# ronnymilleo/amcpy

Hardware: AMD Instinct MI355X
Metric: IQ frames/sec (18 features, 2048-sample complex64) (higher is better)
Workload: dtype f32; 1 GPU; 6 mods x 26 SNR x 4096 frames x 2048 samples complex64 per GPU (BASELINE configs[1]), resident in HBM; one launch per step; frame_size=2048, kernel=amcx_features18_wave_kernel<2048>

## Files before the change

amcpy_amd/_lib.py:

```python
from __future__ import annotations

import ctypes as C
import os
from pathlib import Path

_HERE = Path(__file__).resolve().parent
LIB_PATH = Path(os.environ.get("AMCX_LIB", _HERE / "lib" / "libamcx.so"))

ABI_VERSION = 6
NUM_FEATURES = 18
VARIANT_AUTO, VARIANT_BLOCK, VARIANT_WAVE = 0, 1, 2
VARIANTS = {"auto": VARIANT_AUTO, "block": VARIANT_BLOCK, "wave": VARIANT_WAVE}
OK, EINVAL, ENOTSUP, EHIP, ENODEV, ENOMEM, EIO = 0, -1, -2, -3, -4, -5, -6
SRC_C64, SRC_C128, SRC_F32_SPLIT, SRC_F64_SPLIT = 0, 1, 2, 3


class UploadStats(C.Structure):
    _fields_ = [("frames", C.c_int64), ("source_bytes", C.c_int64), ("pcie_bytes", C.c_int64),
                ("chunks", C.c_int32), ("threads", C.c_int32), ("plane_major", C.c_int32), ("from_file", C.c_int32),
                ("seconds", C.c_double), ("seconds_staging", C.c_double), ("seconds_waiting", C.c_double),
                ("seconds_prepare", C.c_double), ("seconds_tail", C.c_double)]


class Placement(C.Structure):
    _fields_ = [("device", C.c_int32), ("numa_node", C.c_int32), ("n_cpus", C.c_int32), ("n_cpus_allowed", C.c_int32),
                ("first_cpu", C.c_int32), ("last_cpu", C.c_int32), ("pci_bus_id", C.c_char * 32)]


_i64, _i32, _vp, _fp = C.c_int64, C.c_int32, C.c_void_p, C.POINTER(C.c_float)
SIGNATURES = {
    "amcx_abi_version": (C.c_int, []),
    "amcx_strerror": (C.c_char_p, [C.c_int]),
    "amcx_last_hip_error": (C.c_char_p, []),
    "amcx_device_count": (C.c_int, []),
    "amcx_features18_c64": (C.c_int, [_vp, _i64, _i32, _i64, _vp, _i64, _vp]),
    "amcx_features18_c64_ex": (C.c_int, [_vp, _i64, _i32, _i64, _vp, _i64, _vp, _i32]),
    "amcx_features18_workspace_bytes": (_i64, [_i32, _i64, _i32]),
    "amcx_features18_c64_ws": (C.c_int, [_vp, _i64, _i32, _i64, _vp, _i64, _vp, _i32, _vp, _i64]),
    "amcx_features18_c64_host": (C.c_int, [_vp, _i64, _i32, _i64, _vp, _i64, _i32, _i32]),
    "amcx_features18_c128_host": (C.c_int, [_vp, _i64, _i32, _i64, _vp, _i64, _i32, _i32]),
    "amcx_ctx_create": (C.c_int, [_i32, C.POINTER(_vp)]),
    "amcx_ctx_destroy": (C.c_int, [_vp]),
    "amcx_ctx_features18_c64_host": (C.c_int, [_vp, _vp, _i64, _i32, _i64, _vp, _i64, _i32]),
    "amcx_ctx_features18_c128_host": (C.c_int, [_vp, _vp, _i64, _i32, _i64, _vp, _i64, _i32]),
    "amcx_ctx_features18_strided_host": (C.c_int, [_vp, _vp, _vp, _i32, _i64, _i64, _i32, _i64, _i64, _i64,
                                                   _vp, _i64, _i32]),
    "amcx_stage_host": (C.c_int, [_vp, _vp, _i32, _i64, _i64, _i32, _i64, _i64, _i64, _i64, _i64, _vp, _i64, _i32,
                                  C.POINTER(_i32), C.POINTER(_i32)]),
    "amcx_ctx_features18_strided_file": (C.c_int, [_vp, _i32, _i64, _i64, _i32, _i64, _i64, _i32, _i64, _i64, _i64,
                                                   _vp, _i64, _i32]),
    "amcx_stage_file": (C.c_int, [_i32, _i64, _i64, _i32, _i64, _i64, _i32, _i64, _i64, _i64, _i64, _i64, _vp, _i64, _i32,
                                  C.POINTER(_i32), C.POINTER(_i32)]),
    "amcx_ctx_configure": (C.c_int, [_vp, _i32, _i64, _i32]),
    "amcx_ctx_upload_stats": (C.c_int, [_vp, C.POINTER(UploadStats)]),
    "amcx_pack_planes_c64": (C.c_int, [_vp, _i32, _i32, _i64, _i64, _i64, _i32, _vp, _i64, _i32, _vp]),
    "amcx_kernel_name": (C.c_int, [_i32, _i32, C.c_char_p, _i32]),
    "amcx_probe_read_bw": (C.c_int, [_vp, _i64, _vp, _vp]),
    "amcx_probe_fma_rate": (C.c_int, [C.c_double, _vp, C.POINTER(C.c_double), C.POINTER(C.c_double)]),
    "amcx_device_pci_bus_id": (C.c_int, [_i32, C.c_char_p, _i32]),
    "amcx_numa_place": (C.c_int, [C.c_char_p, C.c_char_p, C.POINTER(_i32), C.POINTER(_i32), _i32, C.POINTER(_i32)]),
    "amcx_ctx_bind_cpus": (C.c_int, [_vp, C.POINTER(_i32), _i32]),
    "amcx_ctx_placement": (C.c_int, [_vp, C.POINTER(Placement)]),
    "amcx_group_stats_f32": (C.c_int, [_vp, _i64, _i64, _i64, _i32, _vp, _vp, _vp]),
    "amcx_select_scale_f32": (C.c_int, [_vp, _i64, _i64, _vp, _i32, _vp, _vp, _vp, _i64, _vp]),
    "amcx_group_stats_workspace_bytes": (_i64, [_i64, _i64, _i32]),
    "amcx_group_stats_ws_f32": (C.c_int, [_vp, _i64, _i64, _i64, _i32, _vp, _vp, _vp, _i64, _vp]),
    "amcx_standardize_workspace_bytes": (_i64, [_i64, _i32]),
    "amcx_standardize_fit_transform_f32": (C.c_int, [_vp, _i64, _i64, _i32, C.POINTER(_i32), _i32, _vp, _i64,
                                                     _vp, _vp, _vp, _i64, _vp]),
}

# ... 149 lines not shown
```

amcpy_amd/csrc/amcx.hip:

```cpp
#include "../../include/amcx.h"

#include <hip/hip_runtime.h>
#include <stdio.h>
#include <stdlib.h>
#include <string.h>
#include <chrono>
#include <new>

#include "amcx_block_kernel.h"
#include "amcx_stream_kernel.h"
#include "amcx_wave_kernel.h"
#include "amcx_quad_kernel.h"
#include "amcx_group_kernel.h"
#include "amcx_short_kernel.h"
#include "amcx_post_kernels.h"
#include "amcx_pack_kernel.h"
#include "amcx_upload.h"

namespace {

thread_local char g_hip_err[256] = "";

int hip_fail(hipError_t e, const char* what) {
  snprintf(g_hip_err, sizeof g_hip_err, "%s: %s", what, hipGetErrorString(e));
// ... 213 lines not shown
    case AMCX_OK: return "ok";
    case AMCX_EINVAL: return "invalid argument (null pointer, negative count, stride or frame_size out of range)";
    case AMCX_ENOTSUP: return "kernel variant does not support this frame_size";
    case AMCX_EHIP: return "HIP runtime error (see amcx_last_hip_error)";
    case AMCX_ENODEV: return "no usable gfx950 device";
    case AMCX_ENOMEM: return "device memory allocation failed";
    case AMCX_EIO: return "reading the container's file failed (see amcx_last_hip_error for the errno text)";
    default: return "unknown amcx error code";
  }
}

const char* amcx_last_hip_error(void) { return g_hip_err; }

int amcx_device_count(void) {
  int n = 0;
  hipError_t e = hipGetDeviceCount(&n);
  if (e == hipErrorNoDevice) return 0;
  if (e != hipSuccess) return hip_fail(e, "hipGetDeviceCount");
  int ok = 0;
  for (int d = 0; d < n; ++d) {
    hipDeviceProp_t p;
    if (hipGetDeviceProperties(&p, d) == hipSuccess && strncmp(p.gcnArchName, "gfx950", 6) == 0) ++ok;
  }
  return ok;
}

int64_t amcx_features18_workspace_bytes(int32_t frame_size, int64_t n_frames, int32_t variant) {
  if (n_frames < 0) return -1;
  const int v = resolve_variant(frame_size, variant);
  if (v < 0) return -1;
  if (v != AMCX_VARIANT_BLOCK || frame_size <= amcx::kBlockMaxN || n_frames == 0) return 0;
  const StreamPlan p = stream_plan(frame_size, n_frames);
  return (p.grid + (p.chirped ? 1 : 0)) * (int64_t)p.M * (int64_t)sizeof(float2);
}

int amcx_features18_c64_ws(const void* iq_dev, int64_t n_frames, int32_t frame_size,
                           int64_t row_stride_elems, float* out_dev, int64_t out_row_stride,
                           void* hip_stream, int32_t variant, void* workspace_dev, int64_t workspace_bytes) {
  if (n_frames < 0 || row_stride_elems < frame_size || out_row_stride < AMCX_NUM_FEATURES)
    return AMCX_EINVAL;
  const int v = resolve_variant(frame_size, variant);
  if (v < 0) return v;
  if (n_frames == 0) return AMCX_OK;
  if (iq_dev == nullptr || out_dev == nullptr) return AMCX_EINVAL;
  if ((reinterpret_cast<uintptr_t>(iq_dev) & 7u) || (reinterpret_cast<uintptr_t>(out_dev) & 3u))
    return AMCX_EINVAL;
  if (on_another_device(iq_dev) || on_another_device(out_dev)) return AMCX_EINVAL;
  hipStream_t stream = static_cast<hipStream_t>(hip_stream);
  const float2* iq = static_cast<const float2*>(iq_dev);
  if (v == AMCX_VARIANT_WAVE) {
    hipError_t e;
    if (frame_size == amcx::quad::kN)
      e = amcx::quad::launch_quad(iq, n_frames, row_stride_elems, out_dev, out_row_stride, stream, cu_count());
    else if (frame_size == amcx::group::G<8>::kN)
      e = amcx::group::launch_group<8>(iq, n_frames, row_stride_elems, out_dev, out_row_stride, stream, cu_count());
    else if (frame_size == amcx::group::G<16>::kN)
      e = amcx::group::launch_group<16>(iq, n_frames, row_stride_elems, out_dev, out_row_stride, stream, cu_count());
    else if (amcx::shortk::short_supports(frame_size))
      e = amcx::shortk::launch_short(iq, n_frames, frame_size, row_stride_elems, out_dev, out_row_stride, stream, cu_count());
    else
      e = amcx::launch_wave(iq, n_frames, frame_size, row_stride_elems, out_dev, out_row_stride, stream, cu_count());
    if (e != hipSuccess) return hip_fail(e, "wave kernel launch");
    return AMCX_OK;
  }
  if (workspace_dev != nullptr && on_another_device(workspace_dev)) return AMCX_EINVAL;
  return launch_block(iq, n_frames, frame_size, row_stride_elems, out_dev, out_row_stride, stream, workspace_dev,
                      workspace_bytes < 0 ? 0 : workspace_bytes);
}

int amcx_features18_c64_ex(const void* iq_dev, int64_t n_frames, int32_t frame_size,
                           int64_t row_stride_elems, float* out_dev, int64_t out_row_stride,
                           void* hip_stream, int32_t variant) {
  const int64_t want = n_frames > 0 && iq_dev != nullptr && out_dev != nullptr && row_stride_elems >= frame_size &&
                               out_row_stride >= AMCX_NUM_FEATURES
                           ? amcx_features18_workspace_bytes(frame_size, n_frames, variant) : 0;
  if (want <= 0)
    return amcx_features18_c64_ws(iq_dev, n_frames, frame_size, row_stride_elems, out_dev, out_row_stride, hip_stream,
                                  variant, nullptr, 0);
  hipStream_t st = static_cast<hipStream_t>(hip_stream);
  hipStreamCaptureStatus cap = hipStreamCaptureStatusNone;
  if (hipStreamIsCapturing(st, &cap) != hipSuccess) { (void)hipGetLastError(); cap = hipStreamCaptureStatusNone; }
  void* ws = nullptr;
  if (cap == hipStreamCaptureStatusNone && hipMallocAsync(&ws, (size_t)want, st) != hipSuccess) {
    (void)hipGetLastError();
    ws = nullptr;
  }
  if (ws == nullptr) {
    static const bool verbose = [] { const char* t = getenv("AMCX_VERBOSE"); return t != nullptr && t[0] != '\0' && t[0] != '0'; }();
    static std::atomic<bool> said{false};
    if (verbose && !said.exchange(true))
      fprintf(stderr, "amcx: frame_size %d runs the DFT by its definition (O(N^2)): %s; amcx_features18_c64_ws with %lld "
                      "bytes of workspace selects the FFT form\n", (int)frame_size,
              cap != hipStreamCaptureStatusNone ? "the stream is being captured" : "hipMallocAsync had no workspace", (long long)want);
  }
// ... 882 lines not shown
```

amcpy_amd/csrc/amcx_wave_kernel.h:

```cpp
#pragma once

#include <type_traits>
#include <utility>

#include "amcx_math.h"

#ifndef AMCX_PRIO_MASK
#define AMCX_PRIO_MASK 7
#endif
#define AMCX_PRIO_OF(b) ((AMCX_PRIO_MASK >> (b)) & 1)

namespace amcx {
namespace wave {

constexpr int kNumSums = 27;
constexpr int kStashStride = 33;

constexpr int kEx1StrideKK = 136, kEx1StrideB = 68;
constexpr int kEx2StrideK2 = 65;
constexpr int kExchangeBytes = (7 * kEx1StrideKK + kEx1StrideB + 64) * 8;
constexpr int kTw2Stride = 15 * 8;
constexpr int kTw3Row = 64 * 8;

template <int N>
struct Cfg {
  static_assert(N == 1024 || N == 2048 || N == 4096, "one wave per frame (128 ... 512: amcx_short_kernel.h; 8192 up: quad / group)");
  static constexpr bool kSplit = N == 4096;
  static constexpr int kFramesPerWave = N == 2048 ? 4 : 8;
  static constexpr int kFlushes = N == 4096 ? 2 : 1;
  static constexpr int kStashBytes = kFramesPerWave * kFlushes * kStashStride * 4;
  static constexpr int kTailChunk = 2;
  static constexpr int kRunFrames = kFramesPerWave;
  static constexpr int kWavesPerWG = kSplit ? 8 : 16;
  static constexpr int kThreads = 64 * kWavesPerWG;
  static constexpr int kTailFrames = kWavesPerWG * kFramesPerWave;
  static constexpr int kRows = N / 128;
  static constexpr int kHeldRows = kRows;
  static constexpr int kFftRows = kSplit ? 16 : kRows;
  static constexpr int kFftN = 128 * kFftRows;
  static constexpr int kPhases = kFftRows >= 8 ? kFftRows / 8 : 1;
  static constexpr int kT2Bytes = 8 * kPhases * kTw2Stride;
  static constexpr int kT3Bytes = kPhases * 2 * 7 * kTw3Row;
  static constexpr int kT4Bytes = kSplit ? 64 * 16 : 0;
  static constexpr int kTableBytes = kT2Bytes + kT3Bytes + kT4Bytes;
  static constexpr int kCounterOffset = kTableBytes + kWavesPerWG * (kExchangeBytes + kStashBytes);
  static constexpr int kLdsBytes = kCounterOffset + 16;
  static_assert(kLdsBytes <= 163840, "one workgroup per CU must fit in 160 KiB of LDS");
  static_assert(kFramesPerWave <= 64, "one frame per lane in the finaliser");
  static_assert(kSplit || 2 * kRows * 64 * 4 <= kExchangeBytes, "|x| parking must fit the exchange buffer");
// ... 483 lines not shown
      a[5] = __builtin_fma(A, Bh, a[5]);
      a[6] += AP;
      a[7] = __builtin_fma(Bh, P, a[7]);
      a[8] = __builtin_fma(AA, A, a[8]);
      a[9] = __builtin_fma(A, BB, a[9]);
      a[10] = __builtin_fma(AA, Bh, a[10]);
      a[11] = __builtin_fma(BB, Bh, a[11]);
      a[12] = __builtin_fma(AA, P, a[12]);
      a[13] = __builtin_fma(X4, P, a[13]);
      a[14] = __builtin_fma(AP, Bh, a[14]);
      if (u & 1) __builtin_amdgcn_sched_barrier(0);
    }
  }
#pragma unroll 1
  for (int off = 32; off >= 1; off >>= 1) {
#pragma unroll
    for (int k = 0; k < 15; ++k) a[k] += __shfl_xor(a[k], off, 64);
  }
#pragma unroll
  for (int k = 0; k < 15; ++k) t[k] = a[k];
}

template <int N>
__device__ __forceinline__ void wave_exact_cumulants(const float2* __restrict__ src, float sc, int h, int lane, bool mine,
                                                     float* __restrict__ dst_row) {
  double t[15];
  wave_exact_moments<N>(src, sc, lane, t);
  if (mine) {
    moment_features(t[0], t[1], t[2], t[3], t[4], t[5], t[6], t[7], t[8], t[9], t[10], t[11], t[12], t[13], t[14], (double)N,
                    [&](int j, int twice_order, double v) { dst_row[j] = (float)__builtin_ldexp(v, h * twice_order); });
  }
}

template <int N>
__device__ __forceinline__ void wave_body(
    const float2* __restrict__ iq, long long n_frames, long long row_stride,
    float* __restrict__ out, long long out_stride AMCX_STAMP_ARG) {
  using C = Cfg<N>;
  constexpr int R = C::kFftRows, ROWS = C::kHeldRows;
  constexpr int kWavesPerWG = C::kWavesPerWG, kThreads = C::kThreads, kTailFrames = C::kTailFrames;
  constexpr int kFramesPerWave = C::kFramesPerWave, kTailChunk = C::kTailChunk;
  extern __shared__ float4 amcx_wave_smem[];
  char* smem = reinterpret_cast<char*>(amcx_wave_smem);
  const int tid = threadIdx.x;
  const int lane = tid & 63;
  const int wave = __builtin_amdgcn_readfirstlane(tid >> 6);
  char* t2 = smem;
  char* t3 = smem + C::kT2Bytes;
  char* t4 = smem + C::kTableBytes - C::kT4Bytes;
  char* ex = smem + C::kTableBytes + wave * kExchangeBytes;
  float* stash = reinterpret_cast<float*>(smem + C::kTableBytes + kWavesPerWG * kExchangeBytes) +
                 wave * (kFramesPerWave * C::kFlushes * kStashStride);

  unsigned* const counters = reinterpret_cast<unsigned*>(smem + C::kCounterOffset);
  if (tid == 0) { counters[0] = 0; counters[1] = 0; }
  constexpr int kQ = C::kRunFrames;
  static_assert(kQ % kFramesPerWave == 0 && kFramesPerWave % kTailChunk == 0, "grabs stay inside a run");
  const long long n_wg = gridDim.x, wg = blockIdx.x;
  const long long full_runs = n_frames / kQ;
  const int rem_frames = (int)(n_frames - full_runs * kQ);
  const long long my_full = full_runs > wg ? (full_runs - wg - 1) / n_wg + 1 : 0;
  const long long slice_len = my_full * kQ + (rem_frames > 0 && full_runs % n_wg == wg ? rem_frames : 0);
  const long long body_len = slice_len > kTailFrames ? (slice_len - kTailFrames) / kFramesPerWave * kFramesPerWave : 0;
  const long long tail_len = slice_len - body_len;
  auto frame_of = [&](long long v) -> long long {
    const long long k = v / kQ;
    return (k * n_wg + wg) * kQ + (v - k * kQ);
  };

  build_fft_tables<C::kFftN>(t2, t3, tid, kThreads);
  if constexpr (C::kSplit) {
    for (int e = tid; e < 128; e += kThreads) {
      float sn, cs;
      sincospif((float)e * (1.0f / 2048.0f), &sn, &cs);
      reinterpret_cast<float2*>(t4)[e] = make_float2(cs, -sn);
    }
  }
  __syncthreads();

  const int kkL = lane >> 3, n3L = lane & 7;
  LaneAddr la;
  la.tw2 = t2 + kkL * kTw2Stride;
  la.tw3 = t3 + lane * 8;
  la.ex1_w = ex + lane * 8;
  la.ex1_r = ex + (kkL * kEx1StrideKK + (n3L & 1) * kEx1StrideB + (n3L >> 1)) * 8;
  la.ex2_w = ex + lane * 8;
  la.ex2_r = ex + (n3L * kEx2StrideK2 + kkL * 8) * 8;
  float* const a_lds = reinterpret_cast<float*>(ex) + lane;

#ifdef AMCX_WAVE_STAMPS
  unsigned long long stamp_acc[kStampSections] = {0, 0, 0, 0, 0, 0, 0, 0};
  unsigned long long stamp_last = __builtin_amdgcn_s_memtime();
  const unsigned long long real0 = __builtin_amdgcn_s_memrealtime();
#endif
  for (;;) {
    long long f0;
    int n_here;
    {
      unsigned got = 0;
      if (lane == 0) got = __hip_atomic_fetch_add(&counters[0], (unsigned)kFramesPerWave, __ATOMIC_RELAXED,
                                                  __HIP_MEMORY_SCOPE_WORKGROUP);
      got = __builtin_amdgcn_readfirstlane(got);
      if ((long long)got < body_len) {
        f0 = frame_of(got);
        const long long left = body_len - got;
        n_here = left < kFramesPerWave ? (int)left : kFramesPerWave;
      } else {
        unsigned t = 0;
        if (lane == 0) t = __hip_atomic_fetch_add(&counters[1], (unsigned)kTailChunk, __ATOMIC_RELAXED,
                                                  __HIP_MEMORY_SCOPE_WORKGROUP);
        t = __builtin_amdgcn_readfirstlane(t);
        if ((long long)t >= tail_len) break;
        f0 = frame_of(body_len + t);
        const long long left = tail_len - t;
        n_here = left < kTailChunk ? (int)left : kTailChunk;
      }
    }

    auto load_frame = [&](float (&xr)[2 * ROWS], float (&xi)[2 * ROWS], long long f) {
      const float2* src = iq + f * row_stride + 2 * lane;
      static_for<ROWS>([&](auto ii) {
        constexpr int i = decltype(ii)::value;
        typedef float v4f __attribute__((ext_vector_type(4)));
        const v4f* p = reinterpret_cast<const v4f*>(src + 128 * i);
        const v4f v = __builtin_nontemporal_load(p);
        xr[2 * i] = v.x; xi[2 * i] = v.y; xr[2 * i + 1] = v.z; xi[2 * i + 1] = v.w;
      });
    };
    auto frame = [&](const float (&xr)[2 * ROWS], const float (&xi)[2 * ROWS], int g) {
      asm volatile("; MARK load");
      __builtin_amdgcn_s_setprio(AMCX_PRIO_OF(0));
      AMCX_STAMP(7);
      auto reduce_sums = [&](float (&r28)[28], float (&r7)[7]) __attribute__((always_inline)) {
        asm volatile(
            "s_nop 1\n\t"
            "v_permlane32_swap_b32 %0, %1\n\tv_permlane32_swap_b32 %2, %3\n\t"
            "v_permlane32_swap_b32 %4, %5\n\tv_permlane32_swap_b32 %6, %7\n\t"
            "v_permlane32_swap_b32 %8, %9\n\tv_permlane32_swap_b32 %10, %11\n\t"
            "v_permlane32_swap_b32 %12, %13\n\tv_permlane32_swap_b32 %14, %15\n\t"
            "v_permlane32_swap_b32 %16, %17\n\tv_permlane32_swap_b32 %18, %19\n\t"
            "v_permlane32_swap_b32 %20, %21\n\tv_permlane32_swap_b32 %22, %23\n\t"
            "v_permlane32_swap_b32 %24, %25\n\tv_permlane32_swap_b32 %26, %27"
            : "+v"(r28[0]), "+v"(r28[1]), "+v"(r28[2]), "+v"(r28[3]), "+v"(r28[4]), "+v"(r28[5]),
              "+v"(r28[6]), "+v"(r28[7]), "+v"(r28[8]), "+v"(r28[9]), "+v"(r28[10]), "+v"(r28[11]),
              "+v"(r28[12]), "+v"(r28[13]), "+v"(r28[14]), "+v"(r28[15]), "+v"(r28[16]), "+v"(r28[17]),
              "+v"(r28[18]), "+v"(r28[19]), "+v"(r28[20]), "+v"(r28[21]), "+v"(r28[22]), "+v"(r28[23]),
              "+v"(r28[24]), "+v"(r28[25]), "+v"(r28[26]), "+v"(r28[27]));
        float r14[14];
// ... 22 lines not shown
      };
      auto store_sums = [&](const float (&r7)[7], float* row) __attribute__((always_inline)) {
        int ln = lane;
        asm volatile("" : "+v"(ln));
        if ((ln & 15) == 0) {
          const int rsel = ln >> 4;
          float* dst = row + (((rsel & 1) << 1) | (rsel >> 1));
          static_for<7>([&](auto jj) {
            constexpr int j = decltype(jj)::value;
            dst[4 * j] = r7[j];
          });
        }
      };

      Stats S;
      float sa_flushed = 0.f;
      {
        static_for<ROWS>([&](auto ii) {
          constexpr int i = decltype(ii)::value;
          float a0, a1;
          S.template row<i == 0, i == ROWS - 1>(xr[2 * i], xi[2 * i], xr[2 * i + 1], xi[2 * i + 1], lane, a0, a1);
          if constexpr (!C::kSplit) {
            a_lds[(2 * i) * 64] = a0;
            a_lds[(2 * i + 1) * 64] = a1;
          }
          if constexpr (C::kFlushes == 2 && i == ROWS / 2 - 1) {
            __builtin_amdgcn_sched_barrier(0);
            sa_flushed += S.sa;
            float r28[28] = {S.sA, S.sBh, S.sP, S.sAA, S.sX4, S.sAB, S.sAP, S.sBP, S.sAAA, S.sABB,
                             S.sAAB, S.sBBB, S.sAAP, S.sX4P, S.sABP, S.sa, 0.f, 0.f, 0.f,
                             S.st1, S.st2, S.sab1, S.sab2, S.sw1, S.sw2, S.sw3, S.sw4, 0.f};
            float q7[7];
            reduce_sums(r28, q7);
            store_sums(q7, stash + (g * C::kFlushes) * kStashStride);
            S.clear_sums();
            __builtin_amdgcn_sched_barrier(0);
          }
        });
      }
      asm volatile("; MARK envelope");
      __builtin_amdgcn_s_setprio(AMCX_PRIO_OF(1));
      AMCX_STAMP(0);
      __builtin_amdgcn_sched_barrier(0);
      const float mu = bcast_l63(wave_sum_l63(S.sa + sa_flushed)) * (1.0f / (float)N);
      {
        static_for<2 * ROWS>([&](auto ee) {
          constexpr int e = decltype(ee)::value;
          if constexpr (C::kSplit) {
            S.envelope(__builtin_amdgcn_sqrtf(__builtin_fmaf(xr[e], xr[e], __builtin_fmaf(xi[e], xi[e], kTinyPower))), mu);
          } else {
            S.envelope(a_lds[e * 64], mu);
          }
        });
      }

      asm volatile("; MARK reduce");
      __builtin_amdgcn_s_setprio(AMCX_PRIO_OF(2));
      AMCX_STAMP(3);
      __builtin_amdgcn_sched_barrier(0);
      float* const row = stash + (g * C::kFlushes + (C::kFlushes - 1)) * kStashStride;
      float r7[7];
      {
        float r28[28] = {S.sA, S.sBh, S.sP, S.sAA, S.sX4, S.sAB, S.sAP, S.sBP, S.sAAA, S.sABB,
                         S.sAAB, S.sBBB, S.sAAP, S.sX4P, S.sABP, S.sa, S.sad1, S.sad2, S.sad4,
                         S.st1, S.st2, S.sab1, S.sab2, S.sw1, S.sw2, S.sw3, S.sw4, 0.f};
        reduce_sums(r28, r7);
      }
      const unsigned long long tie = __builtin_amdgcn_ballot_w64(S.wmax > kPi - kTieBand);
      store_sums(r7, row);
      if (lane == 63) {
        row[kNumSums + 1] = S.Kt;
        row[kNumSums + 2] = S.Kw;
        row[kNumSums + 3] = S.Ka;
        row[kNumSums + 4] = tie != 0 ? 1.0f : 0.0f;
      }

      asm volatile("; MARK fft1");
      AMCX_STAMP(1);
      __builtin_amdgcn_sched_barrier(0);
      __builtin_amdgcn_s_setprio(AMCX_PRIO_OF(3));
      float peak;
      if constexpr (!C::kSplit) {
        peak = fft_peak<R>(xr, xi, la);
      } else {
        auto fft4096 = [&](auto&& row_of) -> float {
          const float4 w4 = *reinterpret_cast<const float4*>(t4 + lane * 16);
          float sr[2 * R], si[2 * R], dr[2 * R], di[2 * R];
          if constexpr (AMCX_PRIO_OF(6) != AMCX_PRIO_OF(3)) __builtin_amdgcn_s_setprio(AMCX_PRIO_OF(6));
          static_for<R>([&](auto ii) {
            constexpr int i = decltype(ii)::value;
            constexpr int lo = 2 * i;
            const float4 p = row_of(std::integral_constant<int, i>{});
            const float4 q = row_of(std::integral_constant<int, R + i>{});
// ... 13 lines not shown
            __builtin_amdgcn_s_setprio(AMCX_PRIO_OF(3));
          }
          float s0r[R], s0i[R], s1r[R], s1i[R], d0r[R], d0i[R], d1r[R], d1i[R];
          fft_head<R>(sr, si, s0r, s0i, s1r, s1i);
          const float pk4 = fft_tail<R>(s0r, s0i, s1r, s1i, la, [&](auto gg, auto ww) {
            constexpr int g = decltype(gg)::value, w = decltype(ww)::value;
            if constexpr (g == 0 && w == 0) fft_head<R>(dr, di, d0r, d0i, d1r, d1i);
            if constexpr (g == 0 && w == 1) { dif<8, 0>(d0r, d0i); dif<8, 0>(d1r, d1i); }
            if constexpr (g == 1 && w == 0) { dif<8, 8>(d0r, d0i); dif<8, 8>(d1r, d1i); }
          });
          __builtin_amdgcn_sched_barrier(0);
          return __builtin_fmaxf(pk4, fft_tail<R, true>(d0r, d0i, d1r, d1i, la));
        };
        peak = fft4096([&](auto ic) {
          constexpr int i = decltype(ic)::value;
          return make_float4(xr[2 * i], xi[2 * i], xr[2 * i + 1], xi[2 * i + 1]);
        });
      }

      const float pk = wave_max_l63(peak);
      if (lane == 63) row[kNumSums] = pk;
    };

    auto finalise = [&](auto range_tag, int count) -> unsigned long long {
      constexpr bool RG = decltype(range_tag)::value;
      bool redo = false;
      lds_wave_fence();
      float feat[18];
      long long f = 0;
      [[maybe_unused]] float sc = 1.0f;
      [[maybe_unused]] int ex_half = 0;
      float kw_shift = 0.f;
      bool tie = false, cancel = false;
      if (lane < count) {
        const float* row = stash + (lane * C::kFlushes + (C::kFlushes - 1)) * kStashStride;
        auto sm = [&](int k) -> double {
          double t = row[k];
          if constexpr (C::kFlushes > 1) {
#pragma unroll
            for (int h = 1; h < C::kFlushes; ++h) t += (double)row[k - h * kStashStride];
          }
          return t;
        };
        {
          float s15[15];
#pragma unroll
          for (int k = 0; k < 15; ++k) {
            s15[k] = row[k];
            if constexpr (C::kFlushes > 1) {
#pragma unroll
              for (int h = 1; h < C::kFlushes; ++h) s15[k] += row[k - h * kStashStride];
            }
          }
          cancel = cancellation_suspect(s15, (float)N, (float)cancel_kappa(N));
        }
        FrameSums F;
        F.sA = sm(0); F.sBh = sm(1); F.sP = sm(2); F.sAA = sm(3); F.sX4 = sm(4); F.sAB = sm(5);
        F.sAP = sm(6); F.sBP = sm(7); F.sAAA = sm(8); F.sABB = sm(9); F.sAAB = sm(10);
        F.sBBB = sm(11); F.sAAP = sm(12); F.sX4P = sm(13); F.sABP = sm(14);
        F.sa = sm(15); F.sad1 = sm(16); F.sad2 = sm(17); F.sad4 = sm(18);
        F.std1 = sm(19); F.std2 = sm(20); F.sab1 = sm(21); F.sab2 = sm(22);
        F.swd1 = sm(23); F.swd2 = sm(24); F.swd3 = sm(25); F.swd4 = sm(26);
        F.gmax_raw = row[27]; F.Kt = row[28]; F.Kw = row[29]; F.Ka = row[30];
        F.pi_tie = row[31] != 0.0f;
        kw_shift = row[29];
        if constexpr (RG) {
          const int code = (int)row[kNumSums + 5];
          const int ex = (code >> 6) - 128;
          cancel = finalize_features<true>(F, N, feat, ex) && cancel;
          sc = __builtin_bit_cast(float, (127 - ex) << 23);
          ex_half = ex / 2;
          f = f0 + (code & 63);
        } else {
          cancel = finalize_features(F, N, feat) && cancel;
          if (is_outside_fp32_range(F, N)) redo = true;
          f = f0 + lane;
        }
        cancel = cancel && !redo;
        tie = __builtin_signbitf(feat[4]) && feat[4] == feat[4] && feat[4] != -__builtin_inff() && !redo;
      }
      unsigned long long ties = __builtin_amdgcn_ballot_w64(tie);
      while (ties != 0) {
        const int idx = __builtin_ctzll(ties);
        ties &= ties - 1;
        const unsigned lo = (unsigned)__builtin_amdgcn_readlane((int)(unsigned)(f & 0xffffffffLL), idx);
        const unsigned hi = (unsigned)__builtin_amdgcn_readlane((int)(unsigned)((unsigned long long)f >> 32), idx);
        const long long ft = (long long)(((unsigned long long)hi << 32) | lo);
        float sct = 1.0f;
        if constexpr (RG) sct = __builtin_bit_cast(float, __builtin_amdgcn_readlane(__builtin_bit_cast(int, sc), idx));
        const float kwt = __builtin_bit_cast(float, __builtin_amdgcn_readlane(__builtin_bit_cast(int, kw_shift), idx));
        float f5x, f9x;
        wave_exact_frequency<N>(iq + ft * row_stride, sct, kwt, lane, f5x, f9x);
        if (lane == idx) { feat[4] = f5x; feat[8] = f9x; }
      }
      if (lane < count && !redo) {
        float* dst = out + f * out_stride;
#pragma unroll
        for (int j = 0; j < 18; ++j) dst[j] = feat[j];
      }
      unsigned long long cz = __builtin_amdgcn_ballot_w64(cancel);
      while (cz != 0) {
        const int idx = __builtin_ctzll(cz);
        cz &= cz - 1;
        const unsigned lo = (unsigned)__builtin_amdgcn_readlane((int)(unsigned)(f & 0xffffffffLL), idx);
        const unsigned hi = (unsigned)__builtin_amdgcn_readlane((int)(unsigned)((unsigned long long)f >> 32), idx);
        const long long ft = (long long)(((unsigned long long)hi << 32) | lo);
        float sct = 1.0f;
        int hx = 0;
        if constexpr (RG) {
          sct = __builtin_bit_cast(float, __builtin_amdgcn_readlane(__builtin_bit_cast(int, sc), idx));
          hx = __builtin_amdgcn_readlane(ex_half, idx);
        }
        wave_exact_cumulants<N>(iq + ft * row_stride, sct, hx, lane, lane == idx, out + ft * out_stride);
      }
      lds_wave_fence();
      return __builtin_amdgcn_ballot_w64(redo);
    };

    [[maybe_unused]] const LaneAddr& la_redo = la;
    auto rerun_scaled = [&](unsigned long long todo) {
      while (todo != 0) {
        int cnt = 0;
        for (; cnt < kFramesPerWave && todo != 0; ++cnt) {
          const int idx = __builtin_ctzll(todo);
          todo &= todo - 1;
          float xr[2 * ROWS], xi[2 * ROWS];
          load_frame(xr, xi, f0 + idx);
          float m = 0.f;
          static_for<2 * ROWS>([&](auto ee) {
            constexpr int e = decltype(ee)::value;
            m = __builtin_fmaxf(__builtin_fmaxf(m, __builtin_fabsf(xr[e])), __builtin_fabsf(xi[e]));
          });
          m = bcast_l63(wave_max_l63(m));
          int ex = 0;
          if (m >= 0x1p-125f && m <= 3.4028235e38f) ex = (((__builtin_bit_cast(int, m) >> 23) & 0xff) - 127) & ~1;
          const float sc = __builtin_bit_cast(float, (127 - ex) << 23);
          static_for<2 * ROWS>([&](auto ee) {
            constexpr int e = decltype(ee)::value;
            xr[e] *= sc; xi[e] *= sc;
          });
          frame(xr, xi, cnt);
          if (lane == 63)
            stash[(cnt * C::kFlushes + (C::kFlushes - 1)) * kStashStride + kNumSums + 5] = (float)((ex + 128) * 64 + idx);
        }
        finalise(std::true_type{}, cnt);
      }
    };
    for (int g = 0; g < n_here; ++g) {
      float xr[2 * ROWS], xi[2 * ROWS];
      load_frame(xr, xi, f0 + g);
      frame(xr, xi, g);
    }

    AMCX_STAMP(4);
    asm volatile("; MARK finalize");
    __builtin_amdgcn_s_setprio(AMCX_PRIO_OF(5));
    const unsigned long long left_over = finalise(std::false_type{}, n_here);
    asm volatile("; MARK redo");
    if (left_over != 0) rerun_scaled(left_over);
    AMCX_STAMP(5);
  }
#ifdef AMCX_WAVE_STAMPS
  if (lane == 0) {
    const long long w = (long long)blockIdx.x * kWavesPerWG + wave;
    stamp_acc[6] = __builtin_amdgcn_s_memrealtime() - real0;
#if AMCX_WAVE_STAMPS != 1
    stamp_acc[0] = __builtin_amdgcn_s_memtime() - stamp_last;
#endif
    for (int k = 0; k < kStampSections; ++k) stamp_out[w * kStampSections + k] = stamp_acc[k];
  }
#endif
}

template <int N>
__global__ __launch_bounds__(Cfg<N>::kThreads, (Cfg<N>::kWavesPerWG + 3) / 4) void amcx_features18_wave_kernel(
    const float2* __restrict__ iq, long long n_frames, long long row_stride,
    float* __restrict__ out, long long out_stride AMCX_STAMP_ARG) {
#ifdef AMCX_WAVE_STAMPS
  wave_body<N>(iq, n_frames, row_stride, out, out_stride, stamp_out);
#else
  wave_body<N>(iq, n_frames, row_stride, out, out_stride);
#endif
}

}

inline bool wave_supports(int frame_size) {
  return frame_size >= 128 && frame_size <= 32768 && (frame_size & (frame_size - 1)) == 0;
}

inline const char* wave_kernel_name(int frame_size) {
  switch (frame_size) {
    case 128: return "amcx_features18_short_kernel<128>";
    case 256: return "amcx_features18_short_kernel<256>";
    case 512: return "amcx_features18_short_kernel<512>";
    case 1024: return "amcx_features18_wave_kernel<1024>";
    case 2048: return "amcx_features18_wave_kernel<2048>";
    case 4096: return "amcx_features18_wave_kernel<4096>";
    case 8192: return "amcx_features18_quad_kernel";
    case 16384: return "amcx_features18_group_kernel<8>";
    case 32768: return "amcx_features18_group_kernel<16>";
    default: return "";
  }
}

#ifndef AMCX_WAVE_STAMPS
template <int N>
inline hipError_t launch_wave_n(const float2* iq, int64_t n_frames, int64_t row_stride, float* out,
                                int64_t out_stride, hipStream_t stream, int cus) {
  auto kern = wave::amcx_features18_wave_kernel<N>;
  constexpr int lds = wave::Cfg<N>::kLdsBytes;
  static bool lds_attr_set[64] = {};
  int dev = 0;
  hipError_t e = hipGetDevice(&dev);
  if (e != hipSuccess) return e;
  if (dev < 0 || dev >= 64 || !lds_attr_set[dev]) {
    e = hipFuncSetAttribute(reinterpret_cast<const void*>(kern), hipFuncAttributeMaxDynamicSharedMemorySize, lds);
    if (e != hipSuccess) return e;
    if (dev >= 0 && dev < 64) lds_attr_set[dev] = true;
  }
  int64_t grid = (int64_t)cus;
  const int64_t min_slice = wave::Cfg<N>::kWavesPerWG;
  if (grid * min_slice > n_frames) grid = (n_frames + min_slice - 1) / min_slice;
  hipLaunchKernelGGL(kern, dim3((unsigned)grid), dim3(wave::Cfg<N>::kThreads), lds, stream, iq,
                     (long long)n_frames, (long long)row_stride, out, (long long)out_stride);
  return hipGetLastError();
}

inline hipError_t launch_wave(const float2* iq, int64_t n_frames, int32_t frame_size,
                              int64_t row_stride, float* out, int64_t out_stride,
                              hipStream_t stream, int cus) {
  switch (frame_size) {
    case 1024: return launch_wave_n<1024>(iq, n_frames, row_stride, out, out_stride, stream, cus);
    case 2048: return launch_wave_n<2048>(iq, n_frames, row_stride, out, out_stride, stream, cus);
    case 4096: return launch_wave_n<4096>(iq, n_frames, row_stride, out, out_stride, stream, cus);
    default: return hipErrorNotSupported;
  }
}

#endif

}
```

amcpy_amd/features.py:

```python
from __future__ import annotations

import threading
from typing import Iterable, List

import numpy as np

from . import _lib

FEATURE_IDS = tuple(range(1, _lib.NUM_FEATURES + 1))


def _variant(v) -> int:
    return _lib.VARIANTS[v] if isinstance(v, str) else int(v)


def features18(iq, out=None, *, frame_size: int | None = None, variant="auto"):
    import torch

    _lib.require_torch_runtime()
    if not isinstance(iq, torch.Tensor) or iq.dtype != torch.complex64:
        raise TypeError("iq must be a torch.complex64 tensor")
    if not iq.is_cuda:
        raise ValueError("iq must live in GPU memory (use features18_host for numpy input)")
    if iq.dim() < 1:
        raise ValueError("iq needs at least one dimension")
    L = iq.shape[-1]
    N = L if frame_size is None else int(frame_size)
    if N > L:
        raise ValueError(f"frame_size {N} exceeds row length {L}")
    lead = iq.shape[:-1]
    n_frames = int(np.prod(lead)) if lead else 1
    if iq.stride(-1) != 1 and L > 1:
        raise ValueError("last dimension must have unit stride")
    flat = iq.reshape(n_frames, L) if iq.dim() != 2 else iq
    if flat.data_ptr() != iq.data_ptr() or (n_frames > 1 and flat.stride(1) != 1):
        raise ValueError("frames must be uniformly strided (no copy is made)")
    row_stride = flat.stride(0) if n_frames > 1 else max(L, N)
    if out is None:
        out = torch.empty(lead + (_lib.NUM_FEATURES,), dtype=torch.float32, device=iq.device)
    else:
        if out.dtype != torch.float32 or out.device != iq.device:
            raise TypeError("out must be float32 on the same device")
        if tuple(out.shape[:-1]) != tuple(lead) or out.shape[-1] < _lib.NUM_FEATURES:
            raise ValueError("out must have shape (..., >=18) matching iq")
    oflat = out.reshape(n_frames, out.shape[-1]) if out.dim() != 2 else out
    if oflat.data_ptr() != out.data_ptr() or oflat.stride(-1) != 1:
        raise ValueError("out must be uniformly strided with unit stride in the last dimension")
    out_stride = oflat.stride(0) if n_frames > 1 else out.shape[-1]
    lib = _lib.load()
    v = _variant(variant)
    with torch.cuda.device(iq.device):
        stream = torch.cuda.current_stream(iq.device).cuda_stream
        need = int(lib.amcx_features18_workspace_bytes(N, n_frames, v)) if n_frames > 0 else 0
        if need > 0:
            ws = torch.empty(need, dtype=torch.uint8, device=iq.device)
            _lib.check(lib.amcx_features18_c64_ws(iq.data_ptr(), n_frames, N, row_stride, oflat.data_ptr(), out_stride,
                                                  stream, v, ws.data_ptr(), need))
            ws.record_stream(torch.cuda.current_stream(iq.device))
        else:
            _lib.check(lib.amcx_features18_c64_ex(
                iq.data_ptr(), n_frames, N, row_stride, oflat.data_ptr(), out_stride, stream, v))
    return out[..., :_lib.NUM_FEATURES]


def features18_iq_pairs(iq_pairs, **kw):
    import torch
    if not isinstance(iq_pairs, torch.Tensor) or iq_pairs.dtype != torch.float32 or iq_pairs.shape[-1] != 2:
        raise TypeError("expected a float32 tensor whose last dimension is (I, Q)")
    if iq_pairs.stride(-1) != 1 or (iq_pairs.shape[-2] > 1 and iq_pairs.stride(-2) != 2):
        raise ValueError("(I, Q) pairs must be interleaved in memory")
    return features18(torch.view_as_complex(iq_pairs), **kw)


_tls = threading.local()


def _host_context(device: int) -> "_lib.HostContext":
    cache = getattr(_tls, "ctx", None)
    if cache is None:
        cache = _tls.ctx = {}
    ctx = cache.get(device)
    if ctx is None:
        ctx = cache[device] = _lib.HostContext(device)
    return ctx


# ... 31 lines not shown
```

include/amcx.h:

```cpp
#ifndef AMCX_H_
#define AMCX_H_

#include <stdint.h>

#ifdef __cplusplus
extern "C" {
#endif

#define AMCX_ABI_VERSION 6
#define AMCX_NUM_FEATURES 18

#define AMCX_OK 0
#define AMCX_EINVAL (-1)
#define AMCX_ENOTSUP (-2)
#define AMCX_EHIP (-3)
#define AMCX_ENODEV (-4)
#define AMCX_ENOMEM (-5)
#define AMCX_EIO (-6)

#define AMCX_VARIANT_AUTO 0
#define AMCX_VARIANT_BLOCK 1
#define AMCX_VARIANT_WAVE 2

#define AMCX_MIN_FRAME_SIZE 2
#define AMCX_MAX_FRAME_SIZE 32768
#define AMCX_MAX_BLOCK_FRAME_SIZE 32768

int amcx_abi_version(void);
const char* amcx_strerror(int code);
const char* amcx_last_hip_error(void);
int amcx_device_count(void);

int amcx_features18_c64(const void* iq_dev, int64_t n_frames, int32_t frame_size,
                        int64_t row_stride_elems, float* out_dev, int64_t out_row_stride,
                        void* hip_stream);

int amcx_features18_c64_ex(const void* iq_dev, int64_t n_frames, int32_t frame_size,
                           int64_t row_stride_elems, float* out_dev, int64_t out_row_stride,
                           void* hip_stream, int32_t variant);

int64_t amcx_features18_workspace_bytes(int32_t frame_size, int64_t n_frames, int32_t variant);
int amcx_features18_c64_ws(const void* iq_dev, int64_t n_frames, int32_t frame_size,
                           int64_t row_stride_elems, float* out_dev, int64_t out_row_stride,
                           void* hip_stream, int32_t variant, void* workspace_dev, int64_t workspace_bytes);

int amcx_features18_c64_host(const void* iq_host, int64_t n_frames, int32_t frame_size,
                             int64_t row_stride_elems, float* out_host, int64_t out_row_stride,
                             int32_t device, int32_t variant);

int amcx_features18_c128_host(const void* iq_host, int64_t n_frames, int32_t frame_size,
                              int64_t row_stride_elems, float* out_host, int64_t out_row_stride,
                              int32_t device, int32_t variant);

typedef struct amcx_ctx amcx_ctx;
int amcx_ctx_create(int32_t device, amcx_ctx** ctx_out);
int amcx_ctx_destroy(amcx_ctx* ctx);
int amcx_ctx_features18_c64_host(amcx_ctx* ctx, const void* iq_host, int64_t n_frames,
                                 int32_t frame_size, int64_t row_stride_elems, float* out_host,
                                 int64_t out_row_stride, int32_t variant);
int amcx_ctx_features18_c128_host(amcx_ctx* ctx, const void* iq_host, int64_t n_frames,
                                  int32_t frame_size, int64_t row_stride_elems, float* out_host,
                                  int64_t out_row_stride, int32_t variant);

int amcx_kernel_name(int32_t frame_size, int32_t variant, char* buf, int32_t buf_len);

#define AMCX_SRC_C64 0
#define AMCX_SRC_C128 1
#define AMCX_SRC_F32_SPLIT 2
#define AMCX_SRC_F64_SPLIT 3
int amcx_ctx_features18_strided_host(amcx_ctx* ctx, const void* re, const void* im, int32_t kind,
                                     int64_t n_snr, int64_t n_frames, int32_t frame_size,
                                     int64_t stride_snr, int64_t stride_frame, int64_t stride_sample,
                                     float* out_host, int64_t out_row_stride, int32_t variant);

int amcx_stage_host(const void* re, const void* im, int32_t kind, int64_t n_snr, int64_t n_frames,
                    int32_t frame_size, int64_t stride_snr, int64_t stride_frame, int64_t stride_sample,
                    int64_t first_unit, int64_t n_units, void* dst, int64_t dst_bytes, int32_t threads,
// ... 77 lines not shown
```

Measured before the change: 200.1 million frames/s.

## Batch wave finalize over a global-memory ring of up to 64 frames

For 2048-sample frames, each wave now writes its per-frame partial sums and frame index into a per-wave ring buffer in global workspace instead of the LDS stash. It runs the lane-parallel finalize only when the ring holds up to 64 frames, not after every small grab. The goal is to amortize the finalize/redo phase over a full 64-lane batch so lanes are not left idle on partial batches. In exchange it adds global-memory traffic for the sums, a workspace allocation per call, and extra fence and frame-index bookkeeping.

Measured after the change: 202.5 million frames/s, median of 6. +1.2%, better.

```diff
diff --git a/amcpy_amd/_lib.py b/amcpy_amd/_lib.py
--- a/amcpy_amd/_lib.py
+++ b/amcpy_amd/_lib.py
@@ -7,7 +7,7 @@
 _HERE = Path(__file__).resolve().parent
 LIB_PATH = Path(os.environ.get("AMCX_LIB", _HERE / "lib" / "libamcx.so"))
 
-ABI_VERSION = 6
+ABI_VERSION = 7
 NUM_FEATURES = 18
 VARIANT_AUTO, VARIANT_BLOCK, VARIANT_WAVE = 0, 1, 2
 VARIANTS = {"auto": VARIANT_AUTO, "block": VARIANT_BLOCK, "wave": VARIANT_WAVE}
@@ -37,6 +37,7 @@
     "amcx_features18_c64_ex": (C.c_int, [_vp, _i64, _i32, _i64, _vp, _i64, _vp, _i32]),
     "amcx_features18_workspace_bytes": (_i64, [_i32, _i64, _i32]),
     "amcx_features18_c64_ws": (C.c_int, [_vp, _i64, _i32, _i64, _vp, _i64, _vp, _i32, _vp, _i64]),
+    "amcx_features18_ring_bytes": (_i64, [_i32, _i64, _i32]),
     "amcx_features18_c64_host": (C.c_int, [_vp, _i64, _i32, _i64, _vp, _i64, _i32, _i32]),
     "amcx_features18_c128_host": (C.c_int, [_vp, _i64, _i32, _i64, _vp, _i64, _i32, _i32]),
     "amcx_ctx_create": (C.c_int, [_i32, C.POINTER(_vp)]),
diff --git a/amcpy_amd/csrc/amcx.hip b/amcpy_amd/csrc/amcx.hip
--- a/amcpy_amd/csrc/amcx.hip
+++ b/amcpy_amd/csrc/amcx.hip
@@ -269,6 +269,13 @@
   if (v != AMCX_VARIANT_BLOCK || frame_size <= amcx::kBlockMaxN || n_frames == 0) return 0;
   const StreamPlan p = stream_plan(frame_size, n_frames);
   return (p.grid + (p.chirped ? 1 : 0)) * (int64_t)p.M * (int64_t)sizeof(float2);
+}
+
+int64_t amcx_features18_ring_bytes(int32_t frame_size, int64_t n_frames, int32_t variant) {
+  if (n_frames < 0) return -1;
+  const int v = resolve_variant(frame_size, variant);
+  if (v < 0) return -1;
+  return v == AMCX_VARIANT_WAVE ? amcx::wave_ring_bytes(frame_size, n_frames, cu_count()) : 0;
 }
 
 int amcx_features18_c64_ws(const void* iq_dev, int64_t n_frames, int32_t frame_size,
@@ -295,8 +302,11 @@
       e = amcx::group::launch_group<16>(iq, n_frames, row_stride_elems, out_dev, out_row_stride, stream, cu_count());
     else if (amcx::shortk::short_supports(frame_size))
       e = amcx::shortk::launch_short(iq, n_frames, frame_size, row_stride_elems, out_dev, out_row_stride, stream, cu_count());
-    else
-      e = amcx::launch_wave(iq, n_frames, frame_size, row_stride_elems, out_dev, out_row_stride, stream, cu_count());
+    else {
+      if (workspace_dev != nullptr && on_another_device(workspace_dev)) return AMCX_EINVAL;
+      e = amcx::launch_wave(iq, n_frames, frame_size, row_stride_elems, out_dev, out_row_stride, stream, cu_count(),
+                            workspace_dev, workspace_bytes);
+    }
     if (e != hipSuccess) return hip_fail(e, "wave kernel launch");
     return AMCX_OK;
   }
diff --git a/amcpy_amd/csrc/amcx_wave_kernel.h b/amcpy_amd/csrc/amcx_wave_kernel.h
--- a/amcpy_amd/csrc/amcx_wave_kernel.h
+++ b/amcpy_amd/csrc/amcx_wave_kernel.h
@@ -15,6 +15,8 @@
 
 constexpr int kNumSums = 27;
 constexpr int kStashStride = 33;
+constexpr int kRingStride = 36;
+constexpr int kRingFrameSlot = kNumSums + 7;
 
 constexpr int kEx1StrideKK = 136, kEx1StrideB = 68;
 constexpr int kEx2StrideK2 = 65;
@@ -564,14 +566,18 @@
   }
 }
 
-template <int N>
+template <int N, int B = 0>
 __device__ __forceinline__ void wave_body(
     const float2* __restrict__ iq, long long n_frames, long long row_stride,
-    float* __restrict__ out, long long out_stride AMCX_STAMP_ARG) {
+    float* __restrict__ out, long long out_stride, float* __restrict__ ring AMCX_STAMP_ARG) {
   using C = Cfg<N>;
   constexpr int R = C::kFftRows, ROWS = C::kHeldRows;
   constexpr int kWavesPerWG = C::kWavesPerWG, kThreads = C::kThreads, kTailFrames = C::kTailFrames;
   constexpr int kFramesPerWave = C::kFramesPerWave, kTailChunk = C::kTailChunk;
+  constexpr bool kRing = B > 0;
+  constexpr int kBatch = kRing ? B : kFramesPerWave;
+  constexpr int kRowStride = kRing ? kRingStride : kStashStride;
+  static_assert(!kRing || (B >= kFramesPerWave && B <= 64 && C::kFlushes == 1), "one grab fits the ring; one frame per lane");
   extern __shared__ float4 amcx_wave_smem[];
   char* smem = reinterpret_cast<char*>(amcx_wave_smem);
   const int tid = threadIdx.x;
@@ -581,8 +587,12 @@
   char* t3 = smem + C::kT2Bytes;
   char* t4 = smem + C::kTableBytes - C::kT4Bytes;
   char* ex = smem + C::kTableBytes + wave * kExchangeBytes;
-  float* stash = reinterpret_cast<float*>(smem + C::kTableBytes + kWavesPerWG * kExchangeBytes) +
-                 wave * (kFramesPerWave * C::kFlushes * kStashStride);
+  float* stash;
+  if constexpr (kRing)
+    stash = ring + ((long long)blockIdx.x * kWavesPerWG + wave) * (B * kRingStride);
+  else
+    stash = reinterpret_cast<float*>(smem + C::kTableBytes + kWavesPerWG * kExchangeBytes) +
+            wave * (kFramesPerWave * C::kFlushes * kStashStride);
 
   unsigned* const counters = reinterpret_cast<unsigned*>(smem + C::kCounterOffset);
   if (tid == 0) { counters[0] = 0; counters[1] = 0; }
@@ -625,6 +635,11 @@
   unsigned long long stamp_last = __builtin_amdgcn_s_memtime();
   const unsigned long long real0 = __builtin_amdgcn_s_memrealtime();
 #endif
+  [[maybe_unused]] int fill = 0;
+  [[maybe_unused]] auto store_frame_index = [&](int slot, long long f) {
+    *reinterpret_cast<float2*>(stash + slot * kRingStride + kRingFrameSlot) =
+        make_float2(__builtin_bit_cast(float, (unsigned)f), __builtin_bit_cast(float, (unsigned)((unsigned long long)f >> 32)));
+  };
   for (;;) {
     long long f0;
     int n_here;
@@ -642,10 +657,15 @@
         if (lane == 0) t = __hip_atomic_fetch_add(&counters[1], (unsigned)kTailChunk, __ATOMIC_RELAXED,
                                                   __HIP_MEMORY_SCOPE_WORKGROUP);
         t = __builtin_amdgcn_readfirstlane(t);
-        if ((long long)t >= tail_len) break;
-        f0 = frame_of(body_len + t);
-        const long long left = tail_len - t;
-        n_here = left < kTailChunk ? (int)left : kTailChunk;
+        if ((long long)t >= tail_len) {
+          if constexpr (!kRing) break;
+          f0 = 0;
+          n_here = 0;
+        } else {
+          f0 = frame_of(body_len + t);
+          const long long left = tail_len - t;
+          n_here = left < kTailChunk ? (int)left : kTailChunk;
+        }
       }
     }
 
@@ -734,7 +754,7 @@
                              S.st1, S.st2, S.sab1, S.sab2, S.sw1, S.sw2, S.sw3, S.sw4, 0.f};
             float q7[7];
             reduce_sums(r28, q7);
-            store_sums(q7, stash + (g * C::kFlushes) * kStashStride);
+            store_sums(q7, stash + (g * C::kFlushes) * kRowStride);
             S.clear_sums();
             __builtin_amdgcn_sched_barrier(0);
           }
@@ -760,7 +780,7 @@
       __builtin_amdgcn_s_setprio(AMCX_PRIO_OF(2));
       AMCX_STAMP(3);
       __builtin_amdgcn_sched_barrier(0);
-      float* const row = stash + (g * C::kFlushes + (C::kFlushes - 1)) * kStashStride;
+      float* const row = stash + (g * C::kFlushes + (C::kFlushes - 1)) * kRowStride;
       float r7[7];
       {
         float r28[28] = {S.sA, S.sBh, S.sP, S.sAA, S.sX4, S.sAB, S.sAP, S.sBP, S.sAAA, S.sABB,
@@ -840,8 +860,21 @@
       [[maybe_unused]] int ex_half = 0;
       float kw_shift = 0.f;
       bool tie = false, cancel = false;
+      if constexpr (kRing) __builtin_amdgcn_fence(__ATOMIC_ACQ_REL, "workgroup");
       if (lane < count) {
-        const float* row = stash + (lane * C::kFlushes + (C::kFlushes - 1)) * kStashStride;
+        const float* row;
+        [[maybe_unused]] float rv[kRing ? kRingStride : 1];
+        if constexpr (kRing) {
+          const float4* src = reinterpret_cast<const float4*>(stash + lane * kRingStride);
+#pragma unroll
+          for (int q = 0; q < kRingStride / 4; ++q) {
+            const float4 v = src[q];
+            rv[4 * q] = v.x; rv[4 * q + 1] = v.y; rv[4 * q + 2] = v.z; rv[4 * q + 3] = v.w;
+          }
+          row = rv;
+        } else {
+          row = stash + (lane * C::kFlushes + (C::kFlushes - 1)) * kStashStride;
+        }
         auto sm = [&](int k) -> double {
           double t = row[k];
           if constexpr (C::kFlushes > 1) {
@@ -878,12 +911,15 @@
           cancel = finalize_features<true>(F, N, feat, ex) && cancel;
           sc = __builtin_bit_cast(float, (127 - ex) << 23);
           ex_half = ex / 2;
-          f = f0 + (code & 63);
+          if constexpr (!kRing) f = f0 + (code & 63);
         } else {
           cancel = finalize_features(F, N, feat) && cancel;
           if (is_outside_fp32_range(F, N)) redo = true;
-          f = f0 + lane;
+          if constexpr (!kRing) f = f0 + lane;
         }
+        if constexpr (kRing)
+          f = (long long)(((unsigned long long)__builtin_bit_cast(unsigned, row[kRingFrameSlot + 1]) << 32) |
+                          __builtin_bit_cast(unsigned, row[kRingFrameSlot]));
         cancel = cancel && !redo;
         tie = __builtin_signbitf(feat[4]) && feat[4] == feat[4] && feat[4] != -__builtin_inff() && !redo;
       }
@@ -929,11 +965,17 @@
     auto rerun_scaled = [&](unsigned long long todo) {
       while (todo != 0) {
         int cnt = 0;
-        for (; cnt < kFramesPerWave && todo != 0; ++cnt) {
+        for (; cnt < kBatch && todo != 0; ++cnt) {
           const int idx = __builtin_ctzll(todo);
           todo &= todo - 1;
+          long long fr = f0 + idx;
+          if constexpr (kRing) {
+            const float2 v = *reinterpret_cast<const float2*>(stash + idx * kRingStride + kRingFrameSlot);
+            fr = (long long)(((unsigned long long)(unsigned)__builtin_amdgcn_readfirstlane(__builtin_bit_cast(int, v.y)) << 32) |
+                             (unsigned)__builtin_amdgcn_readfirstlane(__builtin_bit_cast(int, v.x)));
+          }
           float xr[2 * ROWS], xi[2 * ROWS];
-          load_frame(xr, xi, f0 + idx);
+          load_frame(xr, xi, fr);
           float m = 0.f;
           static_for<2 * ROWS>([&](auto ee) {
             constexpr int e = decltype(ee)::value;
@@ -948,25 +990,50 @@
             xr[e] *= sc; xi[e] *= sc;
           });
           frame(xr, xi, cnt);
-          if (lane == 63)
-            stash[(cnt * C::kFlushes + (C::kFlushes - 1)) * kStashStride + kNumSums + 5] = (float)((ex + 128) * 64 + idx);
+          if (lane == 63) {
+            stash[(cnt * C::kFlushes + (C::kFlushes - 1)) * kRowStride + kNumSums + 5] = (float)((ex + 128) * 64 + idx);
+            if constexpr (kRing) store_frame_index(cnt, fr);
+          }
         }
         finalise(std::true_type{}, cnt);
       }
     };
-    for (int g = 0; g < n_here; ++g) {
-      float xr[2 * ROWS], xi[2 * ROWS];
-      load_frame(xr, xi, f0 + g);
-      frame(xr, xi, g);
+    if constexpr (kRing) {
+      if (n_here == 0 || fill + n_here > B) {
+        if (fill > 0) {
+          AMCX_STAMP(4);
+          asm volatile("; MARK finalize");
+          __builtin_amdgcn_s_setprio(AMCX_PRIO_OF(5));
+          const unsigned long long left_over = finalise(std::false_type{}, fill);
+          asm volatile("; MARK redo");
+          if (left_over != 0) rerun_scaled(left_over);
+          AMCX_STAMP(5);
+        }
+        fill = 0;
+        if (n_here == 0) break;
+      }
+      for (int g = 0; g < n_here; ++g) {
+        float xr[2 * ROWS], xi[2 * ROWS];
+        load_frame(xr, xi, f0 + g);
+        frame(xr, xi, fill + g);
+        if (lane == 63) store_frame_index(fill + g, f0 + g);
+      }
+      fill += n_here;
+    } else {
+      for (int g = 0; g < n_here; ++g) {
+        float xr[2 * ROWS], xi[2 * ROWS];
+        load_frame(xr, xi, f0 + g);
+        frame(xr, xi, g);
+      }
+
+      AMCX_STAMP(4);
+      asm volatile("; MARK finalize");
+      __builtin_amdgcn_s_setprio(AMCX_PRIO_OF(5));
+      const unsigned long long left_over = finalise(std::false_type{}, n_here);
+      asm volatile("; MARK redo");
+      if (left_over != 0) rerun_scaled(left_over);
+      AMCX_STAMP(5);
     }
-
-    AMCX_STAMP(4);
-    asm volatile("; MARK finalize");
-    __builtin_amdgcn_s_setprio(AMCX_PRIO_OF(5));
-    const unsigned long long left_over = finalise(std::false_type{}, n_here);
-    asm volatile("; MARK redo");
-    if (left_over != 0) rerun_scaled(left_over);
-    AMCX_STAMP(5);
   }
 #ifdef AMCX_WAVE_STAMPS
   if (lane == 0) {
@@ -985,10 +1052,26 @@
     const float2* __restrict__ iq, long long n_frames, long long row_stride,
     float* __restrict__ out, long long out_stride AMCX_STAMP_ARG) {
 #ifdef AMCX_WAVE_STAMPS
-  wave_body<N>(iq, n_frames, row_stride, out, out_stride, stamp_out);
+  wave_body<N>(iq, n_frames, row_stride, out, out_stride, nullptr, stamp_out);
 #else
-  wave_body<N>(iq, n_frames, row_stride, out, out_stride);
+  wave_body<N>(iq, n_frames, row_stride, out, out_stride, nullptr);
 #endif
+}
+
+template <int N, int B>
+__global__ __launch_bounds__(Cfg<N>::kThreads, (Cfg<N>::kWavesPerWG + 3) / 4) void amcx_features18_wave_kernel(
+    const float2* __restrict__ iq, long long n_frames, long long row_stride,
+    float* __restrict__ out, long long out_stride, float* __restrict__ ring AMCX_STAMP_ARG) {
+#ifdef AMCX_WAVE_STAMPS
+  wave_body<N, B>(iq, n_frames, row_stride, out, out_stride, ring, stamp_out);
+#else
+  wave_body<N, B>(iq, n_frames, row_stride, out, out_stride, ring);
+#endif
+}
+
+template <int N, int B>
+constexpr long long ring_bytes(long long grid) {
+  return grid * Cfg<N>::kWavesPerWG * B * kRingStride * (long long)sizeof(float);
 }
 
 }
@@ -997,6 +1080,9 @@
   return frame_size >= 128 && frame_size <= 32768 && (frame_size & (frame_size - 1)) == 0;
 }
 
+#ifndef AMCX_WAVE_RING
+#define AMCX_WAVE_RING 64
+#endif
 inline const char* wave_kernel_name(int frame_size) {
   switch (frame_size) {
     case 128: return "amcx_features18_short_kernel<128>";
@@ -1014,22 +1100,52 @@
 
 #ifndef AMCX_WAVE_STAMPS
 template <int N>
-inline hipError_t launch_wave_n(const float2* iq, int64_t n_frames, int64_t row_stride, float* out,
-                                int64_t out_stride, hipStream_t stream, int cus) {
-  auto kern = wave::amcx_features18_wave_kernel<N>;
-  constexpr int lds = wave::Cfg<N>::kLdsBytes;
+constexpr int kWaveRingFrames = N == 2048 ? AMCX_WAVE_RING : 0;
+
+template <int N>
+inline int64_t wave_grid(int64_t n_frames, int cus) {
+  int64_t grid = (int64_t)cus;
+  const int64_t min_slice = wave::Cfg<N>::kWavesPerWG;
+  if (grid * min_slice > n_frames) grid = (n_frames + min_slice - 1) / min_slice;
+  return grid;
+}
+
+template <int N, int B>
+inline hipError_t wave_lds_attr(const void* kern) {
   static bool lds_attr_set[64] = {};
   int dev = 0;
   hipError_t e = hipGetDevice(&dev);
   if (e != hipSuccess) return e;
   if (dev < 0 || dev >= 64 || !lds_attr_set[dev]) {
-    e = hipFuncSetAttribute(reinterpret_cast<const void*>(kern), hipFuncAttributeMaxDynamicSharedMemorySize, lds);
+    e = hipFuncSetAttribute(kern, hipFuncAttributeMaxDynamicSharedMemorySize, wave::Cfg<N>::kLdsBytes);
     if (e != hipSuccess) return e;
     if (dev >= 0 && dev < 64) lds_attr_set[dev] = true;
   }
-  int64_t grid = (int64_t)cus;
-  const int64_t min_slice = wave::Cfg<N>::kWavesPerWG;
-  if (grid * min_slice > n_frames) grid = (n_frames + min_slice - 1) / min_slice;
+  return hipSuccess;
+}
+
+inline int64_t wave_ring_bytes(int32_t frame_size, int64_t n_frames, int cus) {
+  if (frame_size != 2048 || kWaveRingFrames<2048> == 0 || n_frames <= 0) return 0;
+  return wave::ring_bytes<2048, kWaveRingFrames<2048>>(wave_grid<2048>(n_frames, cus));
+}
+
+template <int N>
+inline hipError_t launch_wave_n(const float2* iq, int64_t n_frames, int64_t row_stride, float* out,
+                                int64_t out_stride, hipStream_t stream, int cus, void* ws, int64_t ws_bytes) {
+  constexpr int B = kWaveRingFrames<N>, lds = wave::Cfg<N>::kLdsBytes;
+  const int64_t grid = wave_grid<N>(n_frames, cus);
+  hipError_t e;
+  if constexpr (B > 0) {
+    if (ws != nullptr && ws_bytes >= wave::ring_bytes<N, B>(grid) && (reinterpret_cast<uintptr_t>(ws) & 15u) == 0) {
+      auto kern = wave::amcx_features18_wave_kernel<N, B>;
+      if ((e = wave_lds_attr<N, B>(reinterpret_cast<const void*>(kern))) != hipSuccess) return e;
+      hipLaunchKernelGGL(kern, dim3((unsigned)grid), dim3(wave::Cfg<N>::kThreads), lds, stream, iq,
+                         (long long)n_frames, (long long)row_stride, out, (long long)out_stride, static_cast<float*>(ws));
+      return hipGetLastError();
+    }
+  }
+  auto kern = wave::amcx_features18_wave_kernel<N>;
+  if ((e = wave_lds_attr<N, 0>(reinterpret_cast<const void*>(kern))) != hipSuccess) return e;
   hipLaunchKernelGGL(kern, dim3((unsigned)grid), dim3(wave::Cfg<N>::kThreads), lds, stream, iq,
                      (long long)n_frames, (long long)row_stride, out, (long long)out_stride);
   return hipGetLastError();
@@ -1037,11 +1153,11 @@
 
 inline hipError_t launch_wave(const float2* iq, int64_t n_frames, int32_t frame_size,
                               int64_t row_stride, float* out, int64_t out_stride,
-                              hipStream_t stream, int cus) {
+                              hipStream_t stream, int cus, void* ws = nullptr, int64_t ws_bytes = 0) {
   switch (frame_size) {
-    case 1024: return launch_wave_n<1024>(iq, n_frames, row_stride, out, out_stride, stream, cus);
-    case 2048: return launch_wave_n<2048>(iq, n_frames, row_stride, out, out_stride, stream, cus);
-    case 4096: return launch_wave_n<4096>(iq, n_frames, row_stride, out, out_stride, stream, cus);
+    case 1024: return launch_wave_n<1024>(iq, n_frames, row_stride, out, out_stride, stream, cus, ws, ws_bytes);
+    case 2048: return launch_wave_n<2048>(iq, n_frames, row_stride, out, out_stride, stream, cus, ws, ws_bytes);
+    case 4096: return launch_wave_n<4096>(iq, n_frames, row_stride, out, out_stride, stream, cus, ws, ws_bytes);
     default: return hipErrorNotSupported;
   }
 }
diff --git a/amcpy_amd/features.py b/amcpy_amd/features.py
--- a/amcpy_amd/features.py
+++ b/amcpy_amd/features.py
@@ -52,6 +52,8 @@
     with torch.cuda.device(iq.device):
         stream = torch.cuda.current_stream(iq.device).cuda_stream
         need = int(lib.amcx_features18_workspace_bytes(N, n_frames, v)) if n_frames > 0 else 0
+        if need == 0 and n_frames > 0:
+            need = int(lib.amcx_features18_ring_bytes(N, n_frames, v))
         if need > 0:
             ws = torch.empty(need, dtype=torch.uint8, device=iq.device)
             _lib.check(lib.amcx_features18_c64_ws(iq.data_ptr(), n_frames, N, row_stride, oflat.data_ptr(), out_stride,
diff --git a/include/amcx.h b/include/amcx.h
--- a/include/amcx.h
+++ b/include/amcx.h
@@ -7,7 +7,7 @@
 extern "C" {
 #endif
 
-#define AMCX_ABI_VERSION 6
+#define AMCX_ABI_VERSION 7
 #define AMCX_NUM_FEATURES 18
 
 #define AMCX_OK 0
@@ -43,6 +43,8 @@
 int amcx_features18_c64_ws(const void* iq_dev, int64_t n_frames, int32_t frame_size,
                            int64_t row_stride_elems, float* out_dev, int64_t out_row_stride,
                            void* hip_stream, int32_t variant, void* workspace_dev, int64_t workspace_bytes);
+
+int64_t amcx_features18_ring_bytes(int32_t frame_size, int64_t n_frames, int32_t variant);
 
 int amcx_features18_c64_host(const void* iq_host, int64_t n_frames, int32_t frame_size,
                              int64_t row_stride_elems, float* out_host, int64_t out_row_stride,
```
